# BaileyMeche/FM-ReturnPrediction

Hardware: AMD Instinct MI355X
Metric: firm-month rows/sec (and % HBM roofline) for full FM pass at 1/2/4/8 MI355X (higher is better)
Workload: dtype f64; 1 GPU; C3+C4 full pass per GPU: 600 months x 5000 firms x 15 chars; winsorize 1/99 -> NYSE universes -> M1/M2/M3 x 3 universes + Fig-1 x 2 -> NW(4) -> rolling 120/60 -> lagged-rolling forecasts + predictive-slope FM; months_per_gpu=600, firms=5000, chars=15, problems_per_month=11, global_months=600, seed=1, parallelism=month-sharded x1

## Files before the change

### fm-returnprediction_amd/csrc/fm_gram.hip

```cpp
#include <math.h>
#include <stdlib.h>

#include "fm_common.h"
#include "fm_gram_dev.h"

namespace fm {
namespace {

constexpr int GT = 256;
constexpr int GNW = GT / WAVE;
#ifndef FM_GRAM_MINW
#define FM_GRAM_MINW 3
#endif
constexpr int GRAM_MINW = FM_GRAM_MINW;
#ifndef FM_GRAM_WGTIME
#define FM_GRAM_WGTIME 0
#endif
#if FM_GRAM_WGTIME
constexpr int WGT_MAX = 1 << 16;
__device__ uint32_t g_wgtime[4 * WGT_MAX];
#endif

template <int NT, int NB, int MINW, bool PL, bool FULLC>
__global__ __launch_bounds__(GT, MINW) void gram_kernel(fm_gram_args a) {
    using S = GramShape<NT>;
    __shared__ double tile[GNW * S::WT];
    __shared__ double zblk[4 * S::RS];
    __shared__ double prm[4][32];
    __shared__ uint8_t lut[64];

    const int tid = threadIdx.x;
    const int w = __builtin_amdgcn_readfirstlane(tid / WAVE);
    const int ncols = a.ncols, nseg = a.nseg;
    const int nbr = a.npatterns * a.nlevels;
#if FM_GRAM_WGTIME
    const uint64_t t_start = __builtin_amdgcn_s_memrealtime();
#endif
    int c0, c1;
    if (a.wg_chunk_off != nullptr) {
        const int b = (int)gridDim.x - 1 - (int)blockIdx.x;
        c0 = a.wg_chunk_off[b];
        c1 = a.wg_chunk_off[b + 1];
    } else {
        c0 = a.chunk_order ? a.chunk_order[blockIdx.x] : (int)gridDim.x - 1 - (int)blockIdx.x;
        c1 = c0 + 1;
    }
    const int npat = 1 << a.nmodels;
    const int lutv = a.pattern_id[tid < npat ? tid : 0];
    for (int chunk = c0; chunk < c1; ++chunk) {
        const int seg = a.chunk_seg[chunk];
        const int64_t r0 = a.chunk_row[2 * chunk], r1 = a.chunk_row[2 * chunk + 1];
        double pv;
        {
            const int kind = tid >> 5, c = tid & 31;
            const double* src = kind == 0 ? a.lo : kind == 1 ? a.hi : kind == 2 ? a.shift : a.inv_scale;
            const bool on = tid < 128 && c < ncols && src != nullptr;
            const double* pp = on ? src + (int64_t)c * nseg + seg : (const double*)a.seg_off;
            const double v = *pp;
            const double dflt = kind < 2 ? NAN : (kind == 2 ? 0.0 : 1.0);
            pv = on ? v : dflt;
        }
        GramWave<NT, NB, GNW, PL, FULLC> g(a, r0, r1, w);
        g.prefetch();
        if (chunk == c0) {
            for (int e = tid; e < 4 * S::RS; e += GT) zblk[e] = 0.0;
            if (tid < 64) lut[tid] = (uint8_t)lutv;
        }
        if (tid < 128) prm[tid >> 5][tid & 31] = pv;
        __syncthreads();
        g.run(prm, lut, a.inv_scale != nullptr, tile, zblk);
        g.epilogue(tile, a.partial + (int64_t)chunk * nbr * S::PK, nbr);
    }
#if FM_GRAM_WGTIME
    if (tid == 0 && blockIdx.x < WGT_MAX) {
        const uint64_t t_end = __builtin_amdgcn_s_memrealtime();
        uint32_t* f = g_wgtime + 4 * (int64_t)blockIdx.x;
        f[0] = (uint32_t)t_start;
        f[1] = (uint32_t)t_end;
        f[2] = (uint32_t)__builtin_amdgcn_s_getreg((31 << 11) | 4);
        f[3] = (uint32_t)(c1 - c0);
    }
#endif
}

template <int NT, int NB, int MINW>
void launch_gram(const fm_gram_args& a, hipStream_t st) {
    const int grid = a.wg_chunk_off != nullptr ? a.nwg : a.nchunks;
    const bool full = a.ncols == 16 * NT - 1;
    if (a.hi_plane != nullptr) {
        if (full) hipLaunchKernelGGL((gram_kernel<NT, NB, MINW, true, true>), dim3(grid), dim3(GT), 0, st, a);
        else hipLaunchKernelGGL((gram_kernel<NT, NB, MINW, true, false>), dim3(grid), dim3(GT), 0, st, a);
    } else {
        if (full) hipLaunchKernelGGL((gram_kernel<NT, NB, MINW, false, true>), dim3(grid), dim3(GT), 0, st, a);
        else hipLaunchKernelGGL((gram_kernel<NT, NB, MINW, false, false>), dim3(grid), dim3(GT), 0, st, a);
    }
}

}
}

#if FM_GRAM_WGTIME
extern "C" int fm_gram_wgtime_copy(uint32_t* host, int32_t n) {
    return hipMemcpyFromSymbol(host, HIP_SYMBOL(fm::g_wgtime), (size_t)4 * (n < fm::WGT_MAX ? n : fm::WGT_MAX) * 4) ==
                   hipSuccess ? 0 : -1;
}
#endif

extern "C" int fm_gram(const fm_gram_args* args, void* stream) {
    using namespace fm;
    FM_REQUIRE(args != nullptr, "fm_gram: null args");
    const fm_gram_args& a = *args;
    FM_REQUIRE((a.cols || a.hi_plane) && a.seg_off && a.chunk_seg && a.chunk_row && a.partial && a.flags &&
                   a.model_mask && a.model_ymask && a.pattern_id,
               "fm_gram: null pointer");
    FM_REQUIRE(a.ncols >= 1 && a.ncols <= FM_MAX_COLS, "fm_gram: ncols must be 1..%d", FM_MAX_COLS);
    FM_REQUIRE((a.hi_plane == nullptr) == (a.lo_plane == nullptr) && (a.hi_plane == nullptr || a.plane_stride > 0),
               "fm_gram: hi_plane and lo_plane go together (plane_stride > 0)");
    FM_REQUIRE(a.nmodels >= 1 && a.nmodels <= FM_MAX_MODELS, "fm_gram: nmodels must be 1..%d",
               FM_MAX_MODELS);
    FM_REQUIRE(a.nlevels >= 1 && a.nlevels <= FM_MAX_LEVELS, "fm_gram: nlevels must be 1..%d",
               FM_MAX_LEVELS);
    FM_REQUIRE(a.npatterns >= 1, "fm_gram: npatterns must be >= 1");
    if (a.nchunks == 0) return FM_OK;
    FM_REQUIRE(a.wg_chunk_off == nullptr || (a.nwg >= 1 && a.chunk_order == nullptr),
               "fm_gram: a balanced plan needs nwg >= 1 and no chunk_order");
    const int nb = a.npatterns * a.nlevels;
    hipStream_t st = (hipStream_t)stream;
    if (a.ncols <= 15) {
        if (nb <= 1) launch_gram<1, 1, GRAM_MINW>(a, st);
        else if (nb <= 4) launch_gram<1, 4, GRAM_MINW>(a, st);
        else if (nb <= 8) launch_gram<1, 8, GRAM_MINW>(a, st);
        else if (nb <= 12) launch_gram<1, 12, GRAM_MINW>(a, st);
        else if (nb <= 15) launch_gram<1, 15, GRAM_MINW>(a, st);
        else if (nb <= 16) launch_gram<1, 16, GRAM_MINW>(a, st);
        else {
            set_error("fm_gram: %d buckets exceed 16 for <=15 columns", nb);
            return FM_ETOOBIG;
        }
    } else {
        if (nb <= 1) launch_gram<2, 1, 2>(a, st);
        else if (nb <= 4) launch_gram<2, 4, 2>(a, st);
        else if (nb <= 8) launch_gram<2, 8, 2>(a, st);
        else {
            set_error("fm_gram: %d buckets exceed 8 for >15 columns", nb);
            return FM_ETOOBIG;
        }
    }
    FM_CHECK_LAUNCH("fm_gram");
    return FM_OK;
}
```

### fm-returnprediction_amd/csrc/fm_gram_dev.h

```cpp
#pragma once
#include <math.h>

#include "fm_common.h"

namespace fm {
namespace {

__device__ __forceinline__ uint32_t push_valid(uint32_t nn, double x) {
    asm("v_cmp_o_f64 vcc, %1, %1\n\tv_addc_co_u32 %0, vcc, %0, %0, vcc" : "+v"(nn) : "v"(x) : "vcc");
    return nn;
}

template <int CTRL>
__device__ __forceinline__ double dpp_f64(double x) {
    const uint64_t u = (uint64_t)__double_as_longlong(x);
    const uint32_t lo = (uint32_t)__builtin_amdgcn_mov_dpp((int)(uint32_t)u, CTRL, 0xF, 0xF, true);
    const uint32_t hi = (uint32_t)__builtin_amdgcn_mov_dpp((int)(uint32_t)(u >> 32), CTRL, 0xF, 0xF, true);
    return __longlong_as_double((long long)(((uint64_t)hi << 32) | lo));
}

template <int NBLK>
struct BlockPairs {
    static constexpr int P = NBLK * (NBLK + 1) / 2;
    static constexpr int NI = (P + 3) / 4;
    int I[NI * 4], J[NI * 4];
    constexpr BlockPairs() : I(), J() {
        int p = 0;
        for (int i = 0; i < NBLK; ++i)
            for (int j = i; j < NBLK; ++j) {
                I[p] = i;
                J[p] = j;
                ++p;
            }
        for (; p < NI * 4; ++p) I[p] = J[p] = 0;
    }
};

template <int NT>
struct GramShape {
    static constexpr int ZW = 16 * NT;
    static constexpr int RS = ZW + 1;
    static constexpr int TR = WAVE;
    static constexpr int TPAD = 4;
    static constexpr int WT = (TR + TPAD) * RS;
    static constexpr int PK = ZW * (ZW + 1) / 2;
    static constexpr int NI = NT == 1 ? 3 : BlockPairs<8>::NI;
};

template <int NT, int NB, int NWV, bool PL = false, bool FULLC = false>
struct GramWave {
    using S = GramShape<NT>;
    static constexpr int ZW = S::ZW, RS = S::RS, TR = S::TR, WT = S::WT, PK = S::PK, NI = S::NI;

    const fm_gram_args& a;
    int64_t r0, r1;
    int w, lane, ntile;
    double xv[ZW - 1];
    int lv = 0;
    double xw[1];
    int lw = 0;
    double acc[NB][NI];

    __device__ __forceinline__ GramWave(const fm_gram_args& a_, int64_t r0_, int64_t r1_, int w_)
        : a(a_), r0(r0_), r1(r1_), w(w_), lane((int)threadIdx.x & (WAVE - 1)),
          ntile((int)((r1_ - r0_ + TR - 1) / TR)) {}

    __device__ __forceinline__ void load_row(int t) {
        typedef const __attribute__((address_space(1))) char* gptr;
        const int64_t t0 = r0 + (int64_t)t * TR;
        const int64_t last = r1 - 1 - t0;
        const uint32_t lo = last < 0 ? 0u : (last < lane ? (uint32_t)last : (uint32_t)lane);
        const int64_t tb = last < 0 ? r1 - 1 : t0;
        const double* cb = a.cols + tb;
        if constexpr (PL) {
            const uint32_t* hb = a.hi_plane + tb;
            const uint32_t* lb = a.lo_plane + tb;
#pragma unroll
            for (int c = 0; c < ZW - 1; ++c) {
                const uint32_t h = *(const __attribute__((address_space(1))) uint32_t*)((gptr)hb + lo * 4u);
                const uint32_t l = *(const __attribute__((address_space(1))) uint32_t*)((gptr)lb + lo * 4u);
                xv[c] = __longlong_as_double((long long)(((uint64_t)h << 32) | l));
                const int64_t step = FULLC || c + 1 < a.ncols ? a.plane_stride : 0;
                hb += step;
                lb += step;
                asm("" : "+s"(hb), "+s"(lb));
            }
        } else {
#pragma unroll
            for (int c = 0; c < ZW - 1; ++c) {
                xv[c] = *(const __attribute__((address_space(1))) double*)((gptr)cb + lo * 8u);
                cb += FULLC || c + 1 < a.ncols ? a.col_stride : 0;
                asm("" : "+s"(cb));
            }
        }
        const uint8_t* lvbase = a.level ? a.level : (const uint8_t*)a.seg_off;
        lv = *((gptr)(a.level ? lvbase + tb : lvbase) + (a.level ? lo : 0u));
    }

    __device__ __forceinline__ void prefetch() {
        if (w < ntile) load_row(w);
    }

    __device__ __forceinline__ void run(const double (*prm)[32], const uint8_t* lut, bool scaled,
                                        double* tile, const double* zblk) {
        constexpr BlockPairs<4 * NT> BP{};
        const int nmodels = a.nmodels, nlevels = a.nlevels;
        const int lvand = a.level ? 0xFF : 0;
        const uint32_t colmask = a.ncols >= 32 ? ~0u : (1u << a.ncols) - 1u;
#pragma unroll
        for (int b = 0; b < NB; ++b)
#pragma unroll
            for (int k = 0; k < NI; ++k) acc[b][k] = 0.0;
        double* wt = tile + w * WT;
        const int kx = lane & 3, kb = (lane >> 2) & 3, kr = lane >> 4;
        int oa[NI], ob[NI];
#pragma unroll
        for (int k = 0; k < NI; ++k) {
            oa[k] = kr * RS + (NT == 1 ? lane & 15 : 4 * BP.I[4 * k + kb] + kx);
            ob[k] = kr * RS + (NT == 1 ? ((lane & 15) + 4 * k) & 15 : 4 * BP.J[4 * k + kb] + kx);
        }
        const int mmv = (int)a.model_mask[lane < nmodels ? lane : 0];
        uint32_t mm[FM_MAX_MODELS];
#pragma unroll
        for (int m = 0; m < FM_MAX_MODELS; ++m)
            mm[m] = (uint32_t)__builtin_amdgcn_readlane(mmv, m < nmodels ? m : 0);

        auto tile_step = [&](int t, int tnext) {
            const int64_t row = r0 + (int64_t)t * TR + lane;
            uint32_t nn = 0;
#pragma unroll
            for (int c = ZW - 2; c >= 0; --c) nn = push_valid(nn, xv[c]);
            const bool inr = row < r1;
            nn &= inr ? colmask : 0u;
            uint32_t pat = 0;
#pragma unroll
            for (int m = 0; m < FM_MAX_MODELS; ++m)
                if (m < nmodels && (nn & mm[m]) == mm[m]) pat |= 1u << m;
            const int pid = inr ? (int)lut[pat] : 255;
            const int lvm = lv & lvand;
            const int lvl = lvm < nlevels ? lvm : nlevels - 1;
            const int bucket = pid != 255 ? pid * nlevels + lvl : -1;
            constexpr int KB = NB <= 1 ? 0 : NB <= 2 ? 1 : NB <= 4 ? 2 : NB <= 8 ? 3 : 4;
            const bool valid = bucket >= 0;
            const uint64_t bv = __ballot(valid);
            uint64_t bit[KB > 0 ? KB : 1];
#pragma unroll
            for (int i = 0; i < KB; ++i) bit[i] = __ballot(valid && ((bucket >> i) & 1));
            uint32_t eql = (uint32_t)bv, eqh = (uint32_t)(bv >> 32), ltl = 0, lth = 0;
#pragma unroll
            for (int i = KB - 1; i >= 0; --i) {
                const uint32_t tm = 0u - (uint32_t)((bucket >> i) & 1);
                const uint32_t bl = (uint32_t)bit[i], bh = (uint32_t)(bit[i] >> 32);
                ltl |= eql & ~bl & tm;
                lth |= eqh & ~bh & tm;
                eql &= ~(bl ^ tm);
                eqh &= ~(bh ^ tm);
            }
            const int dest = __popc(ltl) + __popc(lth) +
                             (int)__builtin_amdgcn_mbcnt_hi(eqh, __builtin_amdgcn_mbcnt_lo(eql, 0u));
            if (valid) {
                double* dst = wt + dest * RS;
                dst[0] = 1.0;
                if (scaled) {
#pragma unroll
                    for (int c = 0; c < ZW - 1; ++c)
                        dst[1 + c] = (hw_min(hw_max(xv[c], prm[0][c]), prm[1][c]) - prm[2][c]) * prm[3][c];
                } else {
#pragma unroll
                    for (int c = 0; c < ZW - 1; ++c)
                        dst[1 + c] = hw_min(hw_max(xv[c], prm[0][c]), prm[1][c]) - prm[2][c];
                }
            }
            if (tnext < ntile) load_row(tnext);
            __builtin_amdgcn_fence(__ATOMIC_RELEASE, "wavefront");
            __builtin_amdgcn_wave_barrier();
            __builtin_amdgcn_fence(__ATOMIC_ACQUIRE, "wavefront");
            if constexpr (NT == 1) {
                const int abase = (lane >> 4) * RS + (lane & 15);
                const double* rd = wt + abase;
                double An = rd[0];
                int off = 0;
#pragma unroll
                for (int b = 0; b < NB; ++b) {
                    uint64_t mb = bv;
#pragma unroll
                    for (int i = 0; i < KB; ++i) mb &= ((b >> i) & 1) ? bit[i] : ~bit[i];
                    const int n = (int)__popcll(mb);
                    auto group = [&](int g, const double cur, double& nxt) {
                        const int rn = g + 4 < n ? off + g + 4 : off + n;
                        nxt = rd[rn * RS];
                        const double A = kr < n - g ? cur : 0.0;
                        const double B1 = dpp_f64<0x12C>(A), B2 = dpp_f64<0x128>(A);
                        acc[b][0] = __builtin_amdgcn_mfma_f64_4x4x4f64(A, A, acc[b][0], 0, 0, 0);
                        acc[b][1] = __builtin_amdgcn_mfma_f64_4x4x4f64(A, B1, acc[b][1], 0, 0, 0);
                        acc[b][2] = __builtin_amdgcn_mfma_f64_4x4x4f64(A, B2, acc[b][2], 0, 0, 0);
                    };
                    for (int g = 0; g < n; g += 4) {
                        const double Ar = An;
                        group(g, Ar, An);
                    }
                    off += n;
                }
            } else {
                const double* rp = wt;
#pragma unroll
                for (int b = 0; b < NB; ++b) {
                    uint64_t mb = bv;
#pragma unroll
                    for (int i = 0; i < KB; ++i) mb &= ((b >> i) & 1) ? bit[i] : ~bit[i];
                    const int n = (int)__popcll(mb);
                    int g = 0;
                    for (; g + 4 <= n; g += 4, rp += 4 * RS) {
#pragma unroll
                        for (int k = 0; k < NI; ++k)
                            acc[b][k] = __builtin_amdgcn_mfma_f64_4x4x4f64(rp[oa[k]], rp[ob[k]], acc[b][k], 0, 0, 0);
                    }
                    if (g < n) {
                        const double* bp = g + kr < n ? rp : zblk;
#pragma unroll
                        for (int k = 0; k < NI; ++k)
                            acc[b][k] = __builtin_amdgcn_mfma_f64_4x4x4f64(bp[oa[k]], bp[ob[k]], acc[b][k], 0, 0, 0);
                        rp += (n - g) * RS;
                    }
                }
            }
            __builtin_amdgcn_fence(__ATOMIC_RELEASE, "wavefront");
            __builtin_amdgcn_wave_barrier();
            __builtin_amdgcn_fence(__ATOMIC_ACQUIRE, "wavefront");
        };
        for (int t = w; t < ntile; t += NWV) tile_step(t, t + NWV);
    }

    __device__ __forceinline__ void epilogue(double* tile, double* outp, int nbr) {
        constexpr BlockPairs<4 * NT> BP{};
        constexpr int NBATCH = (NWV * WT) / (NWV * PK) < NB ? (NWV * WT) / (NWV * PK) : NB;
        static_assert(NBATCH >= 1, "epilogue image does not fit the tile area");
        const int kx = lane & 3, kb = (lane >> 2) & 3, kr = lane >> 4;
        const int tid = (int)threadIdx.x;
        int od[NI];
#pragma unroll
        for (int k = 0; k < NI; ++k) {
            int r, c;
            bool keep;
            if (NT == 1) {
                r = 4 * kb + kr;
                c = 4 * ((kb + k) & 3) + kx;
                keep = !(k == 2 && kb >= 2) && !(k == 0 && kr > kx);
            } else {
                const int p = 4 * k + kb;
                r = 4 * BP.I[p] + kr;
                c = 4 * BP.J[p] + kx;
                keep = p < BlockPairs<8>::P && !(BP.I[p] == BP.J[p] && kr > kx);
            }
            const int i = r < c ? r : c, j = r < c ? c : r;
            od[k] = keep ? i * ZW - (i * (i - 1)) / 2 + (j - i) : -1;
        }
        __syncthreads();
#pragma unroll
        for (int b0 = 0; b0 < NB; b0 += NBATCH) {
            if (b0 >= nbr) break;
#pragma unroll
            for (int bb = 0; bb < NBATCH; ++bb) {
                const int b = b0 + bb;
                if (b >= NB) continue;
                double* img = tile + (w * NBATCH + bb) * PK;
#pragma unroll
                for (int k = 0; k < NI; ++k)
                    if (od[k] >= 0) img[od[k]] = acc[b][k];
            }
            __syncthreads();
            for (int e = tid; e < NBATCH * PK; e += NWV * WAVE) {
                const int bb = e / PK, f = e - bb * PK;
                const int b = b0 + bb;
                if (b < nbr) {
                    double s = tile[bb * PK + f];
#pragma unroll
                    for (int ww = 1; ww < NWV; ++ww) s += tile[(ww * NBATCH + bb) * PK + f];
                    outp[(int64_t)b * PK + f] = s;
                }
            }
            __syncthreads();
        }
    }
};

}
}
```

### fm-returnprediction_amd/fmcore/_lib.py

```python
from __future__ import annotations

import ctypes as C
import os

_PKG_DIR = os.path.dirname(os.path.dirname(os.path.abspath(__file__)))
LIB_PATH = os.environ.get("FM_HIP_LIB", os.path.join(_PKG_DIR, "lib", "libfm_hip.so"))

FM_ST_FITTED = 0x1
FM_ST_SKIPPED = 0x2
FM_ST_INF_IN_X = 0x4
FM_ST_INF_IN_Y = 0x8
FM_ST_CONST_SUSPECT = 0x10
FM_ST_CONST_COL = 0x20
FM_ST_RANK_DEF = 0x40
FM_ST_REFIT = 0x80

FM_MAX_COLS = 31
FM_MAX_MODELS = 6
FM_MAX_LEVELS = 3
FM_MAX_PORTS = 20
FM_MAX_SORTS = 16
FM_MAX_SORT_K = 30
FM_MAX_DIST_Q = 8
FM_TS_FUSED_MAX_LDS = 128 * 1024
FM_RANK_AVERAGE, FM_RANK_MIN, FM_RANK_MAX = 0, 1, 2
FM_RANK_RAW, FM_RANK_PCT, FM_RANK_UNIFORM = 0, 1, 2

_p = C.c_void_p
_i32 = C.c_int32
_i64 = C.c_int64
_f64 = C.c_double


class GramArgs(C.Structure):
    _fields_ = [
        ("cols", _p), ("col_stride", _i64), ("ncols", _i32), ("nseg", _i32),
        ("seg_off", _p), ("chunk_seg", _p), ("chunk_row", _p), ("nchunks", _i32),
        ("lo", _p), ("hi", _p), ("shift", _p), ("inv_scale", _p),
        ("level", _p), ("nlevels", _i32),
        ("model_mask", _p), ("model_ymask", _p), ("nmodels", _i32),
        ("pattern_id", _p), ("npatterns", _i32),
        ("partial", _p), ("flags", _p), ("chunk_order", _p),
        ("hi_plane", _p), ("lo_plane", _p), ("plane_stride", _i64),
        ("wg_chunk_off", _p), ("nwg", _i32),
    ]


class SelectArgs(C.Structure):
    _fields_ = [
        ("cols", _p), ("col_stride", _i64), ("ncols", _i32), ("seg_off", _p), ("nseg", _i32),
        ("max_seg_len", _i32), ("row_mask", _p), ("q_lo", _f64), ("q_hi", _f64),
        ("min_count", _i32), ("lerp_mode", _i32), ("lo", _p), ("hi", _p), ("nvalid", _p),
        ("mean", _p), ("sd", _p), ("center", _p), ("level", _p), ("ws", _p),
        ("hi_plane", _p), ("plane_stride", _i64), ("lo_plane", _p),
    ]


class UniverseArgs(C.Structure):
    _fields_ = [
        ("me", _p), ("nyse", _p), ("q_a", _f64), ("q_b", _f64), ("cut_a", _p), ("cut_b", _p),
        ("level", _p),
    ]


class TsArgs(C.Structure):
    _fields_ = [
        ("rec", _p), ("r_seg", _i64), ("r_prob", _i64), ("status", _p), ("s_seg", _i64),
        ("s_prob", _i64), ("nseg", _i32), ("nprob", _i32), ("kmax", _i32), ("nw_lags", _i32),
        ("idx", _p), ("count", _p), ("mean", _p), ("se", _p), ("tstat", _p), ("nobs", _p),
        ("work", _p), ("window", _i32), ("min_periods", _i32), ("pmax", _i32), ("roll", _p),
        ("moments", _p), ("mom_stride", _i32), ("prob_k", _p), ("lag", _i32), ("seg_lo", _i32),
        ("seg_hi", _i32), ("pred", _p), ("pred_status", _p),
        ("sum_p_lo", _i32), ("sum_p_hi", _i32), ("roll_own", _i32), ("pad_ts", _i32),
    ]


class SolveArgs(C.Structure):
    _fields_ = [
        ("partial", _p), ("seg_chunk_off", _p), ("nseg", _i32), ("zw", _i32),
        ("nlevels", _i32), ("npatterns", _i32), ("pattern_models", _p),
        ("nprob", _i32), ("prob_model", _p), ("prob_level", _p), ("prob_z", _p),
        ("prob_nz", _p), ("prob_flags", _p), ("add_back", _p), ("gram_flags", _p),
        ("nmodels", _i32), ("pmax", _i32), ("rec", _p), ("status", _p),
        ("moments", _p), ("mom_stride", _i32), ("ab_ncols", _i32),
        ("fix_cols", _p), ("fix_stride", _i64), ("fix_seg_off", _p), ("fix_lo", _p), ("fix_hi", _p),
        ("fix_shift", _p), ("fix_inv_scale", _p), ("fix_level", _p), ("fix_check_const", _i32),
        ("fix_pad", _i32),
        ("fix_hi_plane", _p), ("fix_lo_plane", _p),
    ]


FM_NFIELDS = 12
FM_NCHARS = 12


class CharsArgs(C.Structure):
    _fields_ = [("ids", _p), ("n", _i64), ("field", _p * FM_NFIELDS), ("out", _p * FM_NCHARS)]


class PortArgs(C.Structure):
    _fields_ = [
        ("forecast", _p), ("ret", _p), ("weight", _p), ("level", _p), ("nyse", _p), ("seg_off", _p),
        ("nseg", _i32), ("max_seg_len", _i32), ("nport", _i32), ("min_level", _i32),
        ("nyse_breakpoints", _i32), ("min_count", _i32), ("q", _f64 * (FM_MAX_PORTS - 1)),
        ("bp", _p), ("port", _p), ("rec", _p), ("cnt", _p), ("status", _p),
    ]


class ForecastSrc(C.Structure):
    _fields_ = [
        ("cols", _p), ("col_stride", _i64), ("hi_plane", _p), ("lo_plane", _p), ("plane_stride", _i64),
        ("lo", _p), ("hi", _p), ("coef", _p), ("forecast_out", _p), ("nrows", _i64),
        ("ncols", _i32), ("coef_stride", _i32), ("nsel", _i32), ("pad_src", _i32),
        ("sel_k", _i32 * FM_MAX_SORTS), ("sel_level", _i32 * FM_MAX_SORTS),
        ("sel_cols", (_i32 * FM_MAX_SORT_K) * FM_MAX_SORTS),
    ]


class FPortArgs(C.Structure):
    _fields_ = [
        ("src", ForecastSrc), ("ret_col", _i32), ("nseg", _i32), ("max_seg_len", _i32), ("nport", _i32),
        ("nyse_breakpoints", _i32), ("min_count", _i32), ("weight", _p), ("level", _p), ("nyse", _p),
        ("seg_off", _p), ("q", _f64 * (FM_MAX_PORTS - 1)), ("bp", _p), ("port", _p), ("rec", _p),
        ("cnt", _p), ("status", _p),
    ]


# ... 112 lines not shown
```

### fm-returnprediction_amd/fmcore/engine.py

```python
from __future__ import annotations

import itertools
from dataclasses import dataclass, field
from typing import List, Optional, Sequence

import numpy as np
import torch

from . import _lib as L

LERP_NUMPY = 0
LERP_PANDAS = 1


def require_device():
    if not torch.cuda.is_available():
        raise RuntimeError("fmcore needs a HIP device (MI355X); none is visible and there is "
                           "no CPU fallback")
    L.load()
    return torch.device("cuda", torch.cuda.current_device())


def _ptr(t):
    return None if t is None else t.data_ptr()
# ... 472 lines not shown


GRAM_SLOTS_PER_CU = 3
GRAM_PLAN_SLOTS = 256 * GRAM_SLOTS_PER_CU


def chunk_policy(total_rows, nseg, max_seg_len, slots=None, min_rows=2048):
    slots = slots or GRAM_PLAN_SLOTS
    if nseg > 0 and nseg < 4 * slots:
        R = -(-int(total_rows) // slots)
        if R >= min_rows:
            return ("balanced", int(R))
    return ("months", default_chunk_rows(total_rows, nseg, max_seg_len))


def make_chunks_balanced(seg_off_h, rows_per_wg, row_origin=0):
    so = np.asarray(seg_off_h, dtype=np.int64)
    T = len(so) - 1
    total = int(so[-1])
    R = int(rows_per_wg)
    first = (-int(row_origin)) % R
    blk = np.arange(first, total, R, dtype=np.int64)
    cuts = np.unique(np.concatenate([so, blk[blk > 0]]))
    starts, ends = cuts[:-1], cuts[1:]
    seg_of = np.searchsorted(so, starts, side="right") - 1
    empty = np.nonzero(np.diff(so) == 0)[0]
    if len(empty):
        starts = np.concatenate([starts, so[empty]])
        ends = np.concatenate([ends, so[empty]])
        seg_of = np.concatenate([seg_of, empty])
        order = np.lexsort((seg_of, starts))
        starts, ends, seg_of = starts[order], ends[order], seg_of[order]
    seg = seg_of.astype(np.int32)
    rows = np.stack([starts, ends], axis=1).reshape(-1).astype(np.int64)
    off = np.zeros(T + 1, dtype=np.int32)
    np.cumsum(np.bincount(seg, minlength=T), out=off[1:])
    blk_of = (int(row_origin) + starts) // R
    brk = np.nonzero(np.diff(blk_of))[0] + 1
    wg_off = np.concatenate([[0], brk, [len(seg)]]).astype(np.int32)
    return seg, rows, off, wg_off


def split_policy(nseg):
    return False


def make_chunks_split(seg_off_h, num=3, den=4, min_rows=256):
    T = len(seg_off_h) - 1
    lens = np.diff(seg_off_h).astype(np.int64)
    two = lens >= min_rows
    nch = np.where(two, 2, 1).astype(np.int64)
    off = np.zeros(T + 1, dtype=np.int32)
    np.cumsum(nch, out=off[1:])
    n = int(off[-1])
    seg = np.repeat(np.arange(T, dtype=np.int32), nch)
    rows = np.empty((n, 2), dtype=np.int64)
    first = off[:-1].astype(np.int64)
    cut = seg_off_h[:-1] + (lens * num) // den
    rows[first, 0] = seg_off_h[:-1]
    rows[first, 1] = np.where(two, cut, seg_off_h[1:])
    sec = first[two] + 1
    rows[sec, 0] = cut[two]
    rows[sec, 1] = seg_off_h[1:][two]
    order = np.concatenate([first[::-1], sec[::-1]]).astype(np.int32)
    return seg, rows.reshape(-1), off, order


def make_chunks(seg_off_h, chunk_rows):
    T = len(seg_off_h) - 1
    lens = np.diff(seg_off_h).astype(np.int64)
    nch = np.maximum(1, -(-lens // chunk_rows)).astype(np.int64)
    seg = np.repeat(np.arange(T, dtype=np.int32), nch)
    k = np.arange(len(seg)) - np.repeat(np.cumsum(nch) - nch, nch)
    L = lens[seg]
    n = nch[seg]
    r0 = seg_off_h[seg] + (k * L) // n
    r1 = seg_off_h[seg] + ((k + 1) * L) // n
    rows = np.stack([r0, r1], axis=1).reshape(-1).astype(np.int64)
    off = np.zeros(T + 1, dtype=np.int32)
    np.cumsum(nch, out=off[1:])
    return seg, rows, off


@dataclass
class _Plan:
    chunk_seg: torch.Tensor
    chunk_row: torch.Tensor
    seg_chunk_off: torch.Tensor
    nchunks: int
    order: Optional[torch.Tensor] = None
    wg_off: Optional[torch.Tensor] = None
    nwg: int = 0


def _chunk_plan(panel: DevicePanel):
    cache = getattr(panel, "_chunk_cache", None)
    if cache is not None:
        return cache
    pol = panel.chunk_policy
    if pol is None and panel.chunk_rows is not None:
        pol = ("months", panel.chunk_rows)
    split = panel.chunk_split
    if split is None:
        split = pol is None and split_policy(panel.nseg)
    if pol is None and not split:
        pol = chunk_policy(panel.nrows, panel.nseg, panel.max_seg_len)
    order = wg = None
    if split:
        seg, rows, off, order = make_chunks_split(panel.seg_off_h)
    elif pol[0] == "balanced":
        seg, rows, off, wg = make_chunks_balanced(panel.seg_off_h, pol[1], panel.row_origin)
    else:
        seg, rows, off = make_chunks(panel.seg_off_h, pol[1])
    dev = panel.device
    t = lambda a: None if a is None else torch.from_numpy(np.ascontiguousarray(a)).to(dev)
    plan = _Plan(t(seg), t(rows), t(off), len(seg), t(order), t(wg), 0 if wg is None else len(wg) - 1)
    panel._chunk_cache = plan
    return plan


@dataclass
class _GroupPlan:
    nmodels: int
    npatterns: int
    nprob: int
    mm: torch.Tensor
    ym: torch.Tensor
    lut: torch.Tensor
    patm: torch.Tensor
    pm: torch.Tensor
    pl: torch.Tensor
    pf: torch.Tensor
    pz: torch.Tensor
    pnz: torch.Tensor
    idx: torch.Tensor


def _group_plans(panel, models, problems, nlevels, cap, const_check, dev):
    key = (tuple((m.y, tuple(m.xs), tuple(m.levels), bool(m.const_check)) for m in models),
           nlevels, cap, bool(const_check), str(dev))
    cache = panel.__dict__.setdefault("_group_cache", {})
    if key in cache:
        return cache[key]
    t = lambda a: torch.from_numpy(np.ascontiguousarray(a)).to(dev)
    plans = []
    for g in group_models(models, nlevels, cap):
        gm = [models[i] for i in g]
        lut, pats = plan_patterns(gm)
        gp = [(k, p) for k, p in enumerate(problems) if p.model in g]
        local = {mi: j for j, mi in enumerate(g)}
        pz = np.zeros((len(gp), 32), dtype=np.int32)
        pnz = np.zeros(len(gp), dtype=np.int32)
        for j, (_, p) in enumerate(gp):
            m = models[p.model]
            z = [0] + [1 + x for x in m.xs] + [1 + m.y]
            pz[j, :len(z)] = z
            pnz[j] = len(z)
        plans.append(_GroupPlan(
            nmodels=len(gm), npatterns=len(pats), nprob=len(gp),
            mm=t(np.array([m.mask for m in gm], dtype=np.int64).astype(np.int32)),
            ym=t(np.array([1 << m.y for m in gm], dtype=np.int32)),
            lut=t(lut),
            patm=t(np.array(pats, dtype=np.int64).astype(np.uint32).view(np.int32)),
            pm=t(np.array([local[p.model] for _, p in gp], dtype=np.int32)),
            pl=t(np.array([p.level for _, p in gp], dtype=np.int32)),
            pf=t(np.array([1 if (models[p.model].const_check and const_check) else 0 for _, p in gp],
                          dtype=np.int32)),
            pz=t(pz), pnz=t(pnz),
            idx=t(np.array([k for k, _ in gp], dtype=np.int64))))
    cache[key] = plans
    return plans


def solve_fix_inline(zw, pmax):
    return zw == 16 and pmax + 1 <= 16


def _solve_group(panel, src, gpl, partial, seg_chunk_off, zw, nlevels, T, pmax, mom_stride, lo, hi,
                 shift, inv_scale, add_back, level, const_check, keep):
    dev = src.device
    ng = gpl.nprob
    rs = pmax + 2
    grec = torch.empty((T, ng, rs), dtype=torch.float64, device=dev)
    gst = torch.empty((T, ng), dtype=torch.int32, device=dev)
    gmom = torch.empty((T, ng, mom_stride), dtype=torch.float64, device=dev)
    sa = L.SolveArgs(
        partial=partial.data_ptr(), seg_chunk_off=seg_chunk_off.data_ptr(), nseg=T, zw=zw,
        nlevels=nlevels, npatterns=gpl.npatterns, pattern_models=gpl.patm.data_ptr(), nprob=ng,
        prob_model=gpl.pm.data_ptr(), prob_level=gpl.pl.data_ptr(), prob_z=gpl.pz.data_ptr(),
        prob_nz=gpl.pnz.data_ptr(), prob_flags=gpl.pf.data_ptr(), add_back=_ptr(add_back),
        gram_flags=None, nmodels=gpl.nmodels, pmax=pmax, rec=grec.data_ptr(),
        status=gst.data_ptr(), moments=_ptr(gmom), mom_stride=mom_stride, ab_ncols=src.ncols)
    inline_fix = solve_fix_inline(zw, pmax)
    if not inline_fix and src.f64 is None:
        src = _source(panel, panel.values())

    def set_fix():
        sa.fix_cols, sa.fix_stride, sa.fix_seg_off = src.ptr, src.stride, panel.seg_off.data_ptr()
        if src.f64 is None:
            sa.fix_hi_plane, sa.fix_lo_plane = src.hp, src.lp
        sa.fix_lo, sa.fix_hi, sa.fix_shift, sa.fix_inv_scale = _ptr(lo), _ptr(hi), _ptr(shift), _ptr(inv_scale)
        sa.fix_level, sa.fix_check_const = _ptr(level), int(bool(const_check))

    if inline_fix:
        set_fix()
    _kcall("fm_solve", "fm_solve", L.C.byref(sa), _stream())
    _remember("fm_solve", "fm_solve", L.SolveArgs.from_buffer_copy(sa), partial, seg_chunk_off, gpl, add_back,
              grec, gst, gmom, src.f64, panel.planes, lo, hi, shift, inv_scale, level, *keep)
    if not inline_fix:
        set_fix()
        _kcall("fm_solve_fixup", "fm_solve_fixup", L.C.byref(sa), _stream())
    return grec, gst, gmom


def _problems(models, nlevels):
    problems = []
    for mi, m in enumerate(models):
        for u in m.levels:
            if u >= nlevels:
                raise ValueError("model level beyond the universe levels provided")
            problems.append(Problem(mi, u, len(m.xs)))
    return problems


def fm_pass(panel: DevicePanel, models: Sequence[Model], level=None, nlevels=1, cuts: Cuts = None,
            shift=None, inv_scale=None, add_back=None, moments=False, cols=None, const_check=True):
    src = _source(panel, cols)
    ncols = src.ncols
    if ncols > L.FM_MAX_COLS:
        raise ValueError(f"at most {L.FM_MAX_COLS} columns per pass")
    dev = src.device
    T = panel.nseg
    zw = 16 if ncols <= 15 else 32
    cap = 16 if zw == 16 else 8
    if shift is None:
        shift = pilot_shift(panel, cols)
    if add_back is None and inv_scale is None:
        add_back = shift
    problems = _problems(models, nlevels)
    pmax = max(2, max(p.K + 1 for p in problems))
    nprob = len(problems)
    rs = pmax + 2
    rec = torch.empty((T, nprob, rs), dtype=torch.float64, device=dev)
    status = torch.empty((T, nprob), dtype=torch.int32, device=dev)
    mom_stride = 1 + (pmax + 1) + (pmax + 1) ** 2
    mom = torch.empty((T, nprob, mom_stride), dtype=torch.float64, device=dev) if moments else None
    plan = _chunk_plan(panel)
    lo = cuts.lo if cuts is not None else None
    hi = cuts.hi if cuts is not None else None
    groups = _group_plans(panel, models, problems, nlevels, cap, const_check, dev)
    for gpl in groups:
        nb = gpl.npatterns * nlevels
        partial = torch.empty((plan.nchunks, nb, zw * (zw + 1) // 2), dtype=torch.float64, device=dev)
        flags = torch.empty((T, gpl.nmodels), dtype=torch.int32, device=dev)
        ga = L.GramArgs(
            cols=src.ptr, col_stride=src.stride if src.f64 is not None else 0, ncols=ncols, nseg=T,
            seg_off=panel.seg_off.data_ptr(), chunk_seg=plan.chunk_seg.data_ptr(),
            chunk_row=plan.chunk_row.data_ptr(), nchunks=plan.nchunks,
            lo=_ptr(lo), hi=_ptr(hi), shift=_ptr(shift), inv_scale=_ptr(inv_scale),
            level=_ptr(level), nlevels=nlevels, model_mask=gpl.mm.data_ptr(),
            model_ymask=gpl.ym.data_ptr(), nmodels=gpl.nmodels, pattern_id=gpl.lut.data_ptr(),
            npatterns=gpl.npatterns, partial=partial.data_ptr(), flags=flags.data_ptr(),
            chunk_order=_ptr(plan.order), hi_plane=src.hp, lo_plane=src.lp, plane_stride=src.pstride,
            wg_chunk_off=_ptr(plan.wg_off), nwg=plan.nwg)
        _kcall("fm_gram", "fm_gram", L.C.byref(ga), _stream())
        _remember("fm_gram", "fm_gram", ga, src.f64, panel.planes, partial, flags, lo, hi, shift, inv_scale, level,
                  plan, gpl)
        grec, gst, gmom = _solve_group(panel, src, gpl, partial, plan.seg_chunk_off, zw, nlevels, T, pmax,
                                       mom_stride, lo, hi, shift, inv_scale, add_back, level,
                                       const_check, (src.f64, panel.planes, flags, lo, hi, shift, inv_scale,
                                                     level, plan))
        if len(groups) == 1:
            rec, status = grec, gst
            mom = gmom if moments else None
        else:
            rec.index_copy_(1, gpl.idx, grec)
            status.index_copy_(1, gpl.idx, gst)
            if moments:
                mom.index_copy_(1, gpl.idx, gmom)
    return FMResult(problems=problems, rec=rec, status=status, pmax=pmax, moments=mom,
                    mom_stride=mom_stride)


def drop_degenerate_months(res: FMResult, models: Sequence[Model], sd):
    bad = ~(sd > 0)
    C = sd.shape[0]
    use = np.zeros((res.nprob, C), dtype=np.float64)
    for k, p in enumerate(res.problems):
        use[k, models[p.model].xs] = 1.0
    hit = _small_tensor(tuple(map(tuple, use)), torch.float64, sd.device) @ bad.to(torch.float64)
    res.status &= ~((hit.t() > 0).to(torch.int32) * L.FM_ST_FITTED)
    return res


@dataclass
class TSIndex:
    idx: torch.Tensor
    count: torch.Tensor


def ts_compact(status, s_seg, s_prob, nseg, nprob):
    dev = status.device
    idx = torch.empty((nprob, nseg), dtype=torch.int32, device=dev)
    cnt = torch.empty(nprob, dtype=torch.int32, device=dev)
    _kcall("fm_ts_compact", "fm_ts_compact", status.data_ptr(), s_seg, s_prob, nseg, nprob, idx.data_ptr(),
           cnt.data_ptr(), _stream())
    return TSIndex(idx, cnt)


def compact_result(res: FMResult):
    T, P = res.status.shape
    return ts_compact(res.status, P, 1, T, P)


@dataclass
class Summary:
    mean: torch.Tensor
    se: torch.Tensor
    tstat: torch.Tensor
    nobs: torch.Tensor


def _sum_outputs(nprob, kmax, dev, sum_range):
    if sum_range is None:
        mean = torch.empty((nprob, kmax), dtype=torch.float64, device=dev)
        se, ts = torch.empty_like(mean), torch.empty_like(mean)
        nobs = torch.empty((nprob, kmax), dtype=torch.int32, device=dev)
    else:
        mean = torch.full((nprob, kmax), -0.0, dtype=torch.float64, device=dev)
        se, ts = mean.clone(), mean.clone()
        nobs = torch.zeros((nprob, kmax), dtype=torch.int32, device=dev)
    return mean, se, ts, nobs


def ts_summary(rec, r_seg, r_prob, ix: TSIndex, nseg, nprob, kmax, nw_lags=4, sum_range=None):
    dev = rec.device
    mean, se, ts, nobs = _sum_outputs(nprob, kmax, dev, sum_range)
    p0, p1 = (0, nprob) if sum_range is None else sum_range
    n = p1 - p0
    if n <= 0:
        return Summary(mean, se, ts, nobs)
    work = torch.empty(n * kmax * (max(nseg, 1) + -(-nseg // 2048) * 28), dtype=torch.float64, device=dev)
    _kcall("fm_ts_summary", "fm_ts_summary", rec.data_ptr() + 8 * p0 * r_prob, r_seg, r_prob,
           ix.idx[p0].data_ptr(), ix.count[p0:].data_ptr(), nseg, n, kmax, nw_lags, mean[p0].data_ptr(),
           se[p0].data_ptr(), ts[p0].data_ptr(), nobs[p0].data_ptr(), work.data_ptr(), _stream())
    return Summary(mean, se, ts, nobs)

# ... 565 lines not shown
```

### include/fm_hip.h

```cpp
#ifndef FM_HIP_H
#define FM_HIP_H

#include <stdint.h>

#ifdef __cplusplus
extern "C" {
#endif

#define FM_OK 0
#define FM_EINVAL (-1)
#define FM_EHIP (-2)
#define FM_ETOOBIG (-3)

#define FM_ST_FITTED 0x1u
#define FM_ST_SKIPPED 0x2u
#define FM_ST_INF_IN_X 0x4u
#define FM_ST_INF_IN_Y 0x8u
#define FM_ST_CONST_SUSPECT 0x10u
#define FM_ST_CONST_COL 0x20u
#define FM_ST_RANK_DEF 0x40u
#define FM_ST_REFIT 0x80u

#define FM_MAX_COLS 31
#define FM_MAX_MODELS 6
#define FM_MAX_LEVELS 3

typedef struct fm_gram_args {
    const double* cols;
    int64_t col_stride;
    int32_t ncols;
    int32_t nseg;
    const int64_t* seg_off;
    const int32_t* chunk_seg;
    const int64_t* chunk_row;
    int32_t nchunks;
    const double* lo;
    const double* hi;
    const double* shift;
    const double* inv_scale;
    const uint8_t* level;
    int32_t nlevels;
    const uint32_t* model_mask;
    const uint32_t* model_ymask;
    int32_t nmodels;
    const uint8_t* pattern_id;
    int32_t npatterns;
    double* partial;
    uint32_t* flags;
    const int32_t* chunk_order;
    const uint32_t* hi_plane;
    const uint32_t* lo_plane;
    int64_t plane_stride;
    const int32_t* wg_chunk_off;
    int32_t nwg;
} fm_gram_args;

typedef struct fm_solve_args {
    const double* partial;
    const int32_t* seg_chunk_off;
    int32_t nseg;
    int32_t zw;
    int32_t nlevels;
    int32_t npatterns;
    const uint32_t* pattern_models;
    int32_t nprob;
    const int32_t* prob_model;
    const int32_t* prob_level;
    const int32_t* prob_z;
    const int32_t* prob_nz;
    const int32_t* prob_flags;
    const double* add_back;
    const uint32_t* gram_flags;
    int32_t nmodels;
    int32_t pmax;
    double* rec;
    uint32_t* status;
    double* moments;
    int32_t mom_stride;
    int32_t ab_ncols;
    const double* fix_cols;
    int64_t fix_stride;
    const int64_t* fix_seg_off;
    const double* fix_lo;
    const double* fix_hi;
    const double* fix_shift;
    const double* fix_inv_scale;
    const uint8_t* fix_level;
    int32_t fix_check_const;
    int32_t fix_pad;
    const uint32_t* fix_hi_plane;
    const uint32_t* fix_lo_plane;
} fm_solve_args;

const char* fm_version(void);
const char* fm_last_error(void);
#define FM_ARG_STRUCTS(X)                                                                     \
    X(fm_gram_args) X(fm_solve_args) X(fm_select_args) X(fm_universe_args) X(fm_ts_args)      \
    X(fm_chars_args) X(fm_port_args) X(fm_rank_args) X(fm_forecast_src) X(fm_fport_args)      \
    X(fm_fdist_args)
int64_t fm_struct_size(const char* name);
int fm_device_arch(char* buf, int32_t len);

int fm_select_cuts(const double* cols, int64_t col_stride, int32_t ncols,
                   const int64_t* seg_off, int32_t nseg, int32_t max_seg_len,
                   const uint8_t* row_mask, double q_lo, double q_hi, int32_t min_count,
                   int32_t lerp_mode, double* lo, double* hi, int32_t* nvalid,
                   double* mean, double* sd, void* ws, void* stream);

int64_t fm_select_ws_bytes(int32_t nseg, int32_t ncols, int32_t max_seg_len);

typedef struct fm_select_args {
    const double* cols;
    int64_t col_stride;
    int32_t ncols;
    const int64_t* seg_off;
    int32_t nseg;
    int32_t max_seg_len;
    const uint8_t* row_mask;
    double q_lo, q_hi;
    int32_t min_count;
    int32_t lerp_mode;
    double* lo;
    double* hi;
    int32_t* nvalid;
    double* mean;
    double* sd;
    double* center;
    uint8_t* level;
    void* ws;
    const uint32_t* hi_plane;
    int64_t plane_stride;
    const uint32_t* lo_plane;
} fm_select_args;

int fm_select(const fm_select_args* args, void* stream);

typedef struct fm_universe_args {
    const double* me;
// ... 290 lines not shown
```

Measured before the change: 12.77 billion firm-month rows/s.

## Pipeline gram chunks per workgroup with packed descriptors and progress-based wave priority

Adds a per-workgroup descriptor table, 32-byte entries for up to four chunks, read through scalar constant loads so chunk metadata costs one load. The kernel now prefetches the next chunk's first rows and parameters during the current chunk's epilogue, and stores the new params before the final epilogue barrier, removing one barrier and the load stall between chunks. Waves also set s_setprio by how much of the workgroup's rows are done, so workgroups further behind get scheduling priority. This adds host-side descriptor construction and more complex control flow, and the priority heuristic may not help.

After: 12.86 billion firm-month rows/s (median of 6 runs). No clear change (+0.7%).

```diff
diff --git a/fm-returnprediction_amd/csrc/fm_gram.hip b/fm-returnprediction_amd/csrc/fm_gram.hip
--- a/fm-returnprediction_amd/csrc/fm_gram.hip
+++ b/fm-returnprediction_amd/csrc/fm_gram.hip
@@ -20,6 +20,31 @@
 constexpr int WGT_MAX = 1 << 16;
 __device__ uint32_t g_wgtime[4 * WGT_MAX];
 #endif
+
+struct GramChunk {
+    int chunk, seg;
+    int64_t r0, r1;
+};
+
+template <class T>
+__device__ __forceinline__ T ld_uniform(const T* p) {
+    return *(const __attribute__((address_space(4))) T*)p;
+}
+
+__device__ __forceinline__ GramChunk desc_chunk(const int32_t* rec, int k, int& count, int& wg_rows) {
+    typedef int32_t entry_t __attribute__((ext_vector_type(FM_GRAM_DESC_WORDS)));
+    static_assert(FM_GRAM_DESC_WORDS == 8, "entry layout: chunk, month, r0, r1 (lo, hi), count, rows");
+    const entry_t e = ld_uniform((const entry_t*)(rec + k * FM_GRAM_DESC_WORDS));
+    count = e[6];
+    wg_rows = e[7];
+    return {e[0], e[1], (int64_t)(((uint64_t)(uint32_t)e[3] << 32) | (uint32_t)e[2]),
+            (int64_t)(((uint64_t)(uint32_t)e[5] << 32) | (uint32_t)e[4])};
+}
+
+__device__ __forceinline__ GramChunk array_chunk(const fm_gram_args& a, int chunk) {
+    return {chunk, ld_uniform(a.chunk_seg + chunk), ld_uniform(a.chunk_row + 2 * chunk),
+            ld_uniform(a.chunk_row + 2 * chunk + 1)};
+}
 
 template <int NT, int NB, int MINW, bool PL, bool FULLC>
 __global__ __launch_bounds__(GT, MINW) void gram_kernel(fm_gram_args a) {
@@ -36,40 +61,63 @@
 #if FM_GRAM_WGTIME
     const uint64_t t_start = __builtin_amdgcn_s_memrealtime();
 #endif
-    int c0, c1;
-    if (a.wg_chunk_off != nullptr) {
-        const int b = (int)gridDim.x - 1 - (int)blockIdx.x;
-        c0 = a.wg_chunk_off[b];
-        c1 = a.wg_chunk_off[b + 1];
+    const int32_t* rec = a.wg_desc;
+    int c0, nch, wg_rows = 0;
+    GramChunk ck;
+    if (rec != nullptr) {
+        rec += (int64_t)blockIdx.x * (FM_GRAM_DESC_CHUNKS * FM_GRAM_DESC_WORDS);
+        ck = desc_chunk(rec, 0, nch, wg_rows);
+        c0 = ck.chunk;
     } else {
-        c0 = a.chunk_order ? a.chunk_order[blockIdx.x] : (int)gridDim.x - 1 - (int)blockIdx.x;
-        c1 = c0 + 1;
-    }
+        if (a.wg_chunk_off != nullptr) {
+            const int b = (int)gridDim.x - 1 - (int)blockIdx.x;
+            c0 = ld_uniform(a.wg_chunk_off + b);
+            nch = ld_uniform(a.wg_chunk_off + b + 1) - c0;
+        } else {
+            c0 = a.chunk_order ? ld_uniform(a.chunk_order + blockIdx.x) : (int)gridDim.x - 1 - (int)blockIdx.x;
+            nch = 1;
+        }
+        if (nch <= 0) return;
+        ck = array_chunk(a, c0);
+    }
+    auto chunk_at = [&](int i) {
+        int n, r;
+        return rec != nullptr && i < FM_GRAM_DESC_CHUNKS ? desc_chunk(rec, i, n, r) : array_chunk(a, c0 + i);
+    };
+    auto load_prm = [&](int seg) {
+        const int kind = tid >> 5, c = tid & 31;
+        const double* src = kind == 0 ? a.lo : kind == 1 ? a.hi : kind == 2 ? a.shift : a.inv_scale;
+        const bool on = tid < 128 && c < ncols && src != nullptr;
+        const double* pp = on ? src + (int64_t)c * nseg + seg : (const double*)a.seg_off;
+        const double v = *pp;
+        const double dflt = kind < 2 ? NAN : (kind == 2 ? 0.0 : 1.0);
+        return on ? v : dflt;
+    };
     const int npat = 1 << a.nmodels;
     const int lutv = a.pattern_id[tid < npat ? tid : 0];
-    for (int chunk = c0; chunk < c1; ++chunk) {
-        const int seg = a.chunk_seg[chunk];
-        const int64_t r0 = a.chunk_row[2 * chunk], r1 = a.chunk_row[2 * chunk + 1];
-        double pv;
-        {
-            const int kind = tid >> 5, c = tid & 31;
-            const double* src = kind == 0 ? a.lo : kind == 1 ? a.hi : kind == 2 ? a.shift : a.inv_scale;
-            const bool on = tid < 128 && c < ncols && src != nullptr;
-            const double* pp = on ? src + (int64_t)c * nseg + seg : (const double*)a.seg_off;
-            const double v = *pp;
-            const double dflt = kind < 2 ? NAN : (kind == 2 ? 0.0 : 1.0);
-            pv = on ? v : dflt;
-        }
-        GramWave<NT, NB, GNW, PL, FULLC> g(a, r0, r1, w);
-        g.prefetch();
-        if (chunk == c0) {
-            for (int e = tid; e < 4 * S::RS; e += GT) zblk[e] = 0.0;
-            if (tid < 64) lut[tid] = (uint8_t)lutv;
-        }
-        if (tid < 128) prm[tid >> 5][tid & 31] = pv;
-        __syncthreads();
+    double pv = load_prm(ck.seg);
+    GramWave<NT, NB, GNW, PL, FULLC> g(a, w);
+    g.pace_total(wg_rows);
+    g.begin(ck.r0, ck.r1);
+    for (int e = tid; e < 4 * S::RS; e += GT) zblk[e] = 0.0;
+    if (tid < 64) lut[tid] = (uint8_t)lutv;
+    if (tid < 128) prm[tid >> 5][tid & 31] = pv;
+    __syncthreads();
+    for (int i = 0; i < nch; ++i) {
+        const bool more = i + 1 < nch;
+        GramChunk nx = ck;
+        if (more) nx = chunk_at(i + 1);
         g.run(prm, lut, a.inv_scale != nullptr, tile, zblk);
-        g.epilogue(tile, a.partial + (int64_t)chunk * nbr * S::PK, nbr);
+        g.pace_done += (int)(ck.r1 - ck.r0);
+        double* outp = a.partial + (int64_t)ck.chunk * nbr * S::PK;
+        if (more) {
+            pv = load_prm(nx.seg);
+            g.begin(nx.r0, nx.r1);
+        }
+        g.epilogue(tile, outp, nbr, [&] {
+            if (more && tid < 128) prm[tid >> 5][tid & 31] = pv;
+        });
+        ck = nx;
     }
 #if FM_GRAM_WGTIME
     if (tid == 0 && blockIdx.x < WGT_MAX) {
@@ -78,7 +126,7 @@
         f[0] = (uint32_t)t_start;
         f[1] = (uint32_t)t_end;
         f[2] = (uint32_t)__builtin_amdgcn_s_getreg((31 << 11) | 4);
-        f[3] = (uint32_t)(c1 - c0);
+        f[3] = (uint32_t)nch;
     }
 #endif
 }
@@ -124,6 +172,7 @@
     if (a.nchunks == 0) return FM_OK;
     FM_REQUIRE(a.wg_chunk_off == nullptr || (a.nwg >= 1 && a.chunk_order == nullptr),
                "fm_gram: a balanced plan needs nwg >= 1 and no chunk_order");
+    FM_REQUIRE(((uintptr_t)a.wg_desc & 31) == 0, "fm_gram: wg_desc must be 32-byte aligned");
     const int nb = a.npatterns * a.nlevels;
     hipStream_t st = (hipStream_t)stream;
     if (a.ncols <= 15) {
diff --git a/fm-returnprediction_amd/csrc/fm_gram_dev.h b/fm-returnprediction_amd/csrc/fm_gram_dev.h
--- a/fm-returnprediction_amd/csrc/fm_gram_dev.h
+++ b/fm-returnprediction_amd/csrc/fm_gram_dev.h
@@ -60,10 +60,31 @@
     double xw[1];
     int lw = 0;
     double acc[NB][NI];
-
-    __device__ __forceinline__ GramWave(const fm_gram_args& a_, int64_t r0_, int64_t r1_, int w_)
-        : a(a_), r0(r0_), r1(r1_), w(w_), lane((int)threadIdx.x & (WAVE - 1)),
-          ntile((int)((r1_ - r0_ + TR - 1) / TR)) {}
+    int pace_q[3] = {0, 0, 0};
+    int pace_done = 0;
+
+    __device__ __forceinline__ void pace_total(int wg_rows) {
+        pace_q[0] = wg_rows / 4;
+        pace_q[1] = wg_rows / 2;
+        pace_q[2] = wg_rows - wg_rows / 4;
+    }
+
+    __device__ __forceinline__ void pace(int rows) const {
+        if (rows < pace_q[0]) __builtin_amdgcn_s_setprio(3);
+        else if (rows < pace_q[1]) __builtin_amdgcn_s_setprio(2);
+        else if (rows < pace_q[2]) __builtin_amdgcn_s_setprio(1);
+        else __builtin_amdgcn_s_setprio(0);
+    }
+
+    __device__ __forceinline__ GramWave(const fm_gram_args& a_, int w_)
+        : a(a_), r0(0), r1(0), w(w_), lane((int)threadIdx.x & (WAVE - 1)), ntile(0) {}
+
+    __device__ __forceinline__ void begin(int64_t r0_, int64_t r1_) {
+        r0 = r0_;
+        r1 = r1_;
+        ntile = (int)((r1_ - r0_ + TR - 1) / TR);
+        if (w < ntile) load_row(w);
+    }
 
     __device__ __forceinline__ void load_row(int t) {
         typedef const __attribute__((address_space(1))) char* gptr;
@@ -97,10 +118,6 @@
         lv = *((gptr)(a.level ? lvbase + tb : lvbase) + (a.level ? lo : 0u));
     }
 
-    __device__ __forceinline__ void prefetch() {
-        if (w < ntile) load_row(w);
-    }
-
     __device__ __forceinline__ void run(const double (*prm)[32], const uint8_t* lut, bool scaled,
                                         double* tile, const double* zblk) {
         constexpr BlockPairs<4 * NT> BP{};
@@ -126,6 +143,7 @@
             mm[m] = (uint32_t)__builtin_amdgcn_readlane(mmv, m < nmodels ? m : 0);
 
         auto tile_step = [&](int t, int tnext) {
+            pace(pace_done + t * TR);
             const int64_t row = r0 + (int64_t)t * TR + lane;
             uint32_t nn = 0;
 #pragma unroll
@@ -231,7 +249,8 @@
         for (int t = w; t < ntile; t += NWV) tile_step(t, t + NWV);
     }
 
-    __device__ __forceinline__ void epilogue(double* tile, double* outp, int nbr) {
+    template <class F>
+    __device__ __forceinline__ void epilogue(double* tile, double* outp, int nbr, F before_last_barrier) {
         constexpr BlockPairs<4 * NT> BP{};
         constexpr int NBATCH = (NWV * WT) / (NWV * PK) < NB ? (NWV * WT) / (NWV * PK) : NB;
         static_assert(NBATCH >= 1, "epilogue image does not fit the tile area");
@@ -279,6 +298,7 @@
                     outp[(int64_t)b * PK + f] = s;
                 }
             }
+            if (b0 + NBATCH >= nbr) before_last_barrier();
             __syncthreads();
         }
     }
diff --git a/fm-returnprediction_amd/fmcore/_lib.py b/fm-returnprediction_amd/fmcore/_lib.py
--- a/fm-returnprediction_amd/fmcore/_lib.py
+++ b/fm-returnprediction_amd/fmcore/_lib.py
@@ -18,6 +18,8 @@
 FM_MAX_COLS = 31
 FM_MAX_MODELS = 6
 FM_MAX_LEVELS = 3
+FM_GRAM_DESC_CHUNKS = 4
+FM_GRAM_DESC_WORDS = 8
 FM_MAX_PORTS = 20
 FM_MAX_SORTS = 16
 FM_MAX_SORT_K = 30
@@ -42,7 +44,7 @@
         ("pattern_id", _p), ("npatterns", _i32),
         ("partial", _p), ("flags", _p), ("chunk_order", _p),
         ("hi_plane", _p), ("lo_plane", _p), ("plane_stride", _i64),
-        ("wg_chunk_off", _p), ("nwg", _i32),
+        ("wg_chunk_off", _p), ("nwg", _i32), ("wg_desc", _p),
     ]
 
 
diff --git a/fm-returnprediction_amd/fmcore/engine.py b/fm-returnprediction_amd/fmcore/engine.py
--- a/fm-returnprediction_amd/fmcore/engine.py
+++ b/fm-returnprediction_amd/fmcore/engine.py
@@ -578,6 +578,32 @@
     return seg, rows, off
 
 
+def make_wg_desc(seg, rows, order=None, wg_off=None):
+    K, W = L.FM_GRAM_DESC_CHUNKS, L.FM_GRAM_DESC_WORDS
+    seg = np.asarray(seg, dtype=np.int32)
+    lohi = np.ascontiguousarray(rows, dtype="<i8").view("<i4").reshape(-1, 4)
+    r = np.asarray(rows, dtype=np.int64).reshape(-1, 2)
+    upto = np.concatenate([[0], np.cumsum(r[:, 1] - r[:, 0])])
+    if wg_off is not None:
+        first = np.asarray(wg_off[:-1], dtype=np.int64)[::-1]
+        cnt = np.diff(np.asarray(wg_off, dtype=np.int64))[::-1]
+    else:
+        first = (np.asarray(order, dtype=np.int64) if order is not None
+                 else np.arange(len(seg) - 1, -1, -1, dtype=np.int64))
+        cnt = np.ones(len(first), dtype=np.int64)
+    total = np.minimum(upto[first + cnt] - upto[first], 2 ** 31 - 1) if len(first) <= GRAM_PLAN_SLOTS else 0 * cnt
+    rec = np.zeros((len(first), K, W), dtype=np.int32)
+    for k in range(K):
+        use = np.nonzero(cnt > k)[0]
+        c = first[use] + k
+        rec[use, k, 0] = c
+        rec[use, k, 1] = seg[c]
+        rec[use, k, 2:6] = lohi[c]
+        rec[use, k, 6] = cnt[use]
+        rec[use, k, 7] = total[use]
+    return rec
+
+
 @dataclass
 class _Plan:
     chunk_seg: torch.Tensor
@@ -587,6 +613,7 @@
     order: Optional[torch.Tensor] = None
     wg_off: Optional[torch.Tensor] = None
     nwg: int = 0
+    wg_desc: Optional[torch.Tensor] = None
 
 
 def _chunk_plan(panel: DevicePanel):
@@ -610,7 +637,8 @@
         seg, rows, off = make_chunks(panel.seg_off_h, pol[1])
     dev = panel.device
     t = lambda a: None if a is None else torch.from_numpy(np.ascontiguousarray(a)).to(dev)
-    plan = _Plan(t(seg), t(rows), t(off), len(seg), t(order), t(wg), 0 if wg is None else len(wg) - 1)
+    plan = _Plan(t(seg), t(rows), t(off), len(seg), t(order), t(wg), 0 if wg is None else len(wg) - 1,
+                 t(make_wg_desc(seg, rows, order, wg)))
     panel._chunk_cache = plan
     return plan
 
@@ -758,7 +786,7 @@
             model_ymask=gpl.ym.data_ptr(), nmodels=gpl.nmodels, pattern_id=gpl.lut.data_ptr(),
             npatterns=gpl.npatterns, partial=partial.data_ptr(), flags=flags.data_ptr(),
             chunk_order=_ptr(plan.order), hi_plane=src.hp, lo_plane=src.lp, plane_stride=src.pstride,
-            wg_chunk_off=_ptr(plan.wg_off), nwg=plan.nwg)
+            wg_chunk_off=_ptr(plan.wg_off), nwg=plan.nwg, wg_desc=_ptr(plan.wg_desc))
         _kcall("fm_gram", "fm_gram", L.C.byref(ga), _stream())
         _remember("fm_gram", "fm_gram", ga, src.f64, panel.planes, partial, flags, lo, hi, shift, inv_scale, level,
                   plan, gpl)
diff --git a/include/fm_hip.h b/include/fm_hip.h
--- a/include/fm_hip.h
+++ b/include/fm_hip.h
@@ -53,7 +53,10 @@
     int64_t plane_stride;
     const int32_t* wg_chunk_off;
     int32_t nwg;
+    const int32_t* wg_desc;
 } fm_gram_args;
+#define FM_GRAM_DESC_CHUNKS 4
+#define FM_GRAM_DESC_WORDS 8
 
 typedef struct fm_solve_args {
     const double* partial;
```
